# suoych/KEDs

Measured on AMD Instinct MI355X. Metric: query-images/sec (encode+0.5M top-10) ViT-L/14, higher is better.
Workload: dtype bf16/fp16 operands, fp32 accumulate; 1 GPU; ViT-L/14 encode_image (224x224 synthetic, random-init weights) + exact top-10 over a synthetic unit-norm 0.5M x 768 database; batch_per_gpu=128, global_batch=128, db_rows=500000, dim=768, k=10, parallelism=dp1 encoders + 1-way row-sharded scan

## Files before the change

### keds_amd/csrc/gemm.hip

```cpp
#include "keds_common.h"
#include <math.h>
#include "gemm_shared.h"
#include "gemm_quad_gen.h"

#ifndef KEDS_QUAD_AUX_X
#define KEDS_QUAD_AUX_X 0
#endif
#ifndef KEDS_QUAD_AUX_W
#define KEDS_QUAD_AUX_W 0
#endif

namespace {

constexpr int BM = 128, BN = 128, BK = 64;
constexpr int TILE_BYTES = 128 * BK * 2;
constexpr int BUF_BYTES = 2 * TILE_BYTES;


__device__ __forceinline__ float qgelu(float x) {
    return x * __builtin_amdgcn_rcpf(1.0f + __builtin_amdgcn_exp2f(-2.4554669595930157f * x));
}

template <int EPI>
__device__ __forceinline__ void epilogue_store(f32x4 v0, f32x4 v1, void* __restrict__ out, int m, int n, int N,
// ... 198 lines not shown
                if (m >= M) continue;
                if constexpr (epi_x3(EPI))
                    epilogue_store<epi_base(EPI)>(acc[2 * p][mi] * x3_ws + b0, acc[2 * p + 1][mi] * x3_ws + b1, out, m, n, N, aux, aux_i, ldc);
                else
                    epilogue_store<epi_base(EPI)>(acc[2 * p][mi] + b0, acc[2 * p + 1][mi] + b1, out, m, n, N, aux, aux_i, ldc, guard);
            }
        }
    }
}

template <int EPI>
constexpr int quad_nd() { return 18; }
template <int EPI, int ND = 0, int H = 0, int PSEL = -1>
__device__ __forceinline__ void pair_ln_epilogue(f32x4 (&acc)[4][8], const char* __restrict__ side, void* __restrict__ out,
                                                 int m0, int n0, int N, int wm, int wn, int g, int c,
                                                 void* __restrict__ aux2, u32x4* __restrict__ pend = nullptr, bool defer = false,
                                                 int* __restrict__ guard = nullptr) {
    float rstd[8], nmr[8];
    [[maybe_unused]] unsigned rmax = 0;
    int r0 = 128 * wm + c;
    asm volatile("" : "+v"(r0));
#pragma unroll
    for (int mi = 0; mi < 8; ++mi) {
        const f32x2 cf = *reinterpret_cast<const f32x2*>(side + (r0 + 16 * mi) * 8);
        rstd[mi] = cf[0];
        nmr[mi] = cf[1];
    }
    if (PSEL <= 0 && aux2 && n0 == 0 && wn == 0 && g == 0) {
        keds_stat_t* zero = reinterpret_cast<keds_stat_t*>(aux2) + 2 * (size_t)(m0 + r0);
#pragma unroll
        for (int mi = 0; mi < 8; ++mi) keds_stat_zero(zero + 32 * mi);
    }
    char* tile_out = reinterpret_cast<char*>(out) + ((size_t)m0 * N + n0) * 2;
#pragma unroll
    for (int p = 0; p < 2; ++p) {
        if (PSEL >= 0 && p != PSEL) continue;
        const int nl = 64 * wn + 32 * p + 8 * g;
        const f32x4 b0 = *reinterpret_cast<const f32x4*>(side + 2048 + nl * 4), b1 = *reinterpret_cast<const f32x4*>(side + 2048 + nl * 4 + 16);
        const f32x4 c0 = *reinterpret_cast<const f32x4*>(side + 3072 + nl * 4), c1 = *reinterpret_cast<const f32x4*>(side + 3072 + nl * 4 + 16);
#pragma unroll
        for (int mi = 0; mi < 8; ++mi) {
            f32x4 v0 = acc[2 * p][mi] * rstd[mi] + (c0 * nmr[mi] + b0);
            f32x4 v1 = acc[2 * p + 1][mi] * rstd[mi] + (c1 * nmr[mi] + b1);
            if constexpr (epi_qgelu(EPI)) {
                f32x4 z0 = v0 * -2.4554669595930157f, z1 = v1 * -2.4554669595930157f;
#pragma unroll
                for (int j = 0; j < 4; ++j) {
                    z0[j] = __builtin_amdgcn_exp2f(z0[j]);
                    z1[j] = __builtin_amdgcn_exp2f(z1[j]);
                }
                z0 = z0 + 1.0f;
                z1 = z1 + 1.0f;
#pragma unroll
                for (int j = 0; j < 4; ++j) {
                    z0[j] = __builtin_amdgcn_rcpf(z0[j]);
                    z1[j] = __builtin_amdgcn_rcpf(z1[j]);
                }
                v0 = v0 * z0;
                v1 = v1 * z1;
            }
            const unsigned off = ((unsigned)(r0 + 16 * mi) * (unsigned)N + (unsigned)nl) * 2u;
            u32x4 ov;
            if constexpr (epi_out_f16(EPI)) {
                rmax = f16_range_max(rmax, v0, v1);
                ov = __builtin_bit_cast(u32x4, f16x8{(f16_t)v0[0], (f16_t)v0[1], (f16_t)v0[2], (f16_t)v0[3],
                                                     (f16_t)v1[0], (f16_t)v1[1], (f16_t)v1[2], (f16_t)v1[3]});
            } else {
                ov = __builtin_bit_cast(u32x4, bf16x8{(bf16_t)v0[0], (bf16_t)v0[1], (bf16_t)v0[2], (bf16_t)v0[3],
                                                      (bf16_t)v1[0], (bf16_t)v1[1], (bf16_t)v1[2], (bf16_t)v1[3]});
            }
            if constexpr (ND > 0) {
                if (16 * H + p * 8 + mi >= 32 - ND && defer) {
                    pend[16 * H + p * 8 + mi - (32 - ND)] = ov;
                    continue;
                }
            }
            keds_store16<KEDS_ST_LN>(ov, tile_out, off);
        }
    }
    if constexpr (epi_out_f16(EPI)) f16_range_flag(guard, rmax);
}
template <int ND>
__device__ __forceinline__ void quad_flush_pending(const u32x4* __restrict__ pend, char* __restrict__ tile_out, int N, int wm, int wn2,
                                                   int g, int c, int i0, int i1) {
    int r0 = 128 * wm + c;
    asm volatile("" : "+v"(r0));
#pragma unroll
    for (int i = 0; i < ND; ++i) {
        if (i < i0 || i >= i1) continue;
        const int s_ = 32 - ND + i, h = s_ >> 4, p = (s_ >> 3) & 1, mi = s_ & 7;
        const unsigned off = ((unsigned)(r0 + 16 * mi) * (unsigned)N + (unsigned)(64 * (2 * wn2 + h) + 32 * p + 8 * g)) * 2u;
        keds_store16<KEDS_ST_LN>(pend[i], tile_out, off);
    }
}

template <bool REDUCE = true>
__device__ __forceinline__ void pair_resid_epilogue(f32x4 (&acc)[4][8], const char* __restrict__ side, void* __restrict__ out,
                                                    int m0, int n0, int N, int wm, int wn, int g, int c,
                                                    keds_stat_t* __restrict__ stats, char* __restrict__ red) {
    const int r0 = 128 * wm + c;
    char* tile = reinterpret_cast<char*>(out) + ((size_t)m0 * N + n0) * 2;
    const int nl = 64 * wn + 8 * g;
    f16x8 r[2][8];
#if KEDS_LD_RESID_AUX
    const auto trs = __builtin_amdgcn_make_buffer_rsrc(tile, 0, 0x7FFFFFFF, 0x00020000);
#endif
#pragma unroll
    for (int p = 0; p < 2; ++p)
#pragma unroll
        for (int mi = 0; mi < 8; ++mi) {
#if KEDS_LD_RESID_AUX
            r[p][mi] = __builtin_bit_cast(f16x8, __builtin_amdgcn_raw_buffer_load_b128(
                           trs, (int)(((unsigned)(r0 + 16 * mi) * (unsigned)N + (unsigned)(nl + 32 * p)) * 2u), 0, KEDS_LD_RESID_AUX));
#else
            r[p][mi] = *reinterpret_cast<const f16x8*>(tile + ((unsigned)(r0 + 16 * mi) * (unsigned)N + (unsigned)(nl + 32 * p)) * 2u);
#endif
        }
    f32x4 b[2][2];
#pragma unroll
    for (int p = 0; p < 2; ++p) {
        b[p][0] = *reinterpret_cast<const f32x4*>(side + 2048 + (nl + 32 * p) * 4);
        b[p][1] = *reinterpret_cast<const f32x4*>(side + 2048 + (nl + 32 * p) * 4 + 16);
    }
    f32x2* rw = reinterpret_cast<f32x2*>(red) + wn * 256 + r0;
#pragma unroll
    for (int mi = 0; mi < 8; ++mi) {
        f32x4 sv = f32x4{0.f, 0.f, 0.f, 0.f}, qv = sv;
#pragma unroll
        for (int p = 0; p < 2; ++p) {
            const f16x8 q = r[p][mi];
            const f32x4 v0 = f32x4{(float)q[0], (float)q[1], (float)q[2], (float)q[3]} + (acc[2 * p][mi] + b[p][0]);
            const f32x4 v1 = f32x4{(float)q[4], (float)q[5], (float)q[6], (float)q[7]} + (acc[2 * p + 1][mi] + b[p][1]);
            const f16x8 ov = f16x8{(f16_t)v0[0], (f16_t)v0[1], (f16_t)v0[2], (f16_t)v0[3], (f16_t)v1[0], (f16_t)v1[1], (f16_t)v1[2], (f16_t)v1[3]};
            keds_store16<KEDS_ST_RESID>(ov, tile, ((unsigned)(r0 + 16 * mi) * (unsigned)N + (unsigned)(nl + 32 * p)) * 2u);
            sv = sv + (v0 + v1);
            qv = qv + (v0 * v0 + v1 * v1);
        }
        float s = (sv[0] + sv[1]) + (sv[2] + sv[3]), ss = (qv[0] + qv[1]) + (qv[2] + qv[3]);
        s = rows_sum(s);
        ss = rows_sum(ss);
        if (stats && g == 0) rw[16 * mi] = f32x2{s, ss};
    }
    if constexpr (REDUCE) {
        if (stats) {
            __syncthreads();
            const int t = threadIdx.x;
            if (t < 256) {
                const f32x2* rr = reinterpret_cast<const f32x2*>(red) + t;
                const f32x2 a = rr[0], b = rr[256], c2 = rr[512], d = rr[768];
                keds_stat_add(stats + 2 * (size_t)(m0 + t), (a[0] + b[0]) + (c2[0] + d[0]), (a[1] + b[1]) + (c2[1] + d[1]));
            }
        }
    }
}

__device__ __forceinline__ void pair_resid_epilogue_acc(f32x4 (&acc)[4][8], void* __restrict__ out, int m0, int n0, int N,
                                                        int wm, int wn, int g, int c, keds_stat_t* __restrict__ stats,
                                                        char* __restrict__ red) {
    const int r0 = 128 * wm + c;
    char* tile = reinterpret_cast<char*>(out) + ((size_t)m0 * N + n0) * 2;
    const int nl = 64 * wn + 8 * g;
    f32x2* rw = reinterpret_cast<f32x2*>(red) + wn * 256 + r0;
#pragma unroll
    for (int mi = 0; mi < 8; ++mi) {
        float s = 0.f, ss = 0.f;
#pragma unroll
        for (int p = 0; p < 2; ++p) {
            const f32x4 v0 = acc[2 * p][mi], v1 = acc[2 * p + 1][mi];
            const f16x8 ov = f16x8{(f16_t)v0[0], (f16_t)v0[1], (f16_t)v0[2], (f16_t)v0[3], (f16_t)v1[0], (f16_t)v1[1], (f16_t)v1[2], (f16_t)v1[3]};
            *reinterpret_cast<f16x8*>(tile + ((unsigned)(r0 + 16 * mi) * (unsigned)N + (unsigned)(nl + 32 * p)) * 2u) = ov;
            s += sum8(v0, v1);
            ss += sum8(v0 * v0, v1 * v1);
        }
        s = rows_sum(s);
        ss = rows_sum(ss);
        if (stats && g == 0) rw[16 * mi] = f32x2{s, ss};
    }
    if (stats) {
        __syncthreads();
        const int t = threadIdx.x;
        if (t < 256) {
            const f32x2* rr = reinterpret_cast<const f32x2*>(red) + t;
            const f32x2 a = rr[0], b = rr[256], c2 = rr[512], d = rr[768];
            keds_stat_add(stats + 2 * (size_t)(m0 + t), (a[0] + b[0]) + (c2[0] + d[0]), (a[1] + b[1]) + (c2[1] + d[1]));
        }
    }
}

template <int N>
__device__ __forceinline__ void small_wait_barrier() {
    asm volatile("s_waitcnt vmcnt(%0)\n\ts_barrier" ::"n"(N) : "memory");
}
template <int MAXAHEAD>
__device__ __forceinline__ void small_wait_stage(int ahead) {
    if constexpr (MAXAHEAD == 0) {
        small_wait_barrier<0>();
    } else {
        if (ahead >= MAXAHEAD) small_wait_barrier<MAXAHEAD * 8>();
        else small_wait_stage<MAXAHEAD - 1>(ahead);
    }
}

template <int EPI, int NST>
__global__ __launch_bounds__(256, 2) void gemm_bt_kernel(const bf16_t* __restrict__ X, const bf16_t* __restrict__ W,
                                                         const float* __restrict__ bias, void* __restrict__ out,
                                                         int M, int N, int K, int n_tiles,
                                                         const float* __restrict__ aux, int aux_i,
                                                         float* __restrict__ part, int k_len, int tiles, int m_pad,
                                                         long long lda, long long ldc, void* __restrict__ aux2,
                                                         int* __restrict__ guard, long long a_plane, long long w_plane) {
    extern __shared__ __attribute__((aligned(16))) char smem[];
    const int bid_all = xcd_remap(blockIdx.x, gridDim.x);
    const int ks = part ? bid_all / tiles : 0;
    const int bid = part ? bid_all - ks * tiles : bid_all;
    const int k_begin = ks * k_len;
    const int tm = bid / n_tiles, tn = bid - tm * n_tiles;
    const int m0 = tm * BM, n0 = tn * BN;
    const int tid = threadIdx.x, lane = tid & 63;
    const int wave = __builtin_amdgcn_readfirstlane(tid >> 6);
    const int wn = wave >> 1, wm = wave & 1;
    const int g = lane >> 4, c = lane & 15;

    const int srow = lane >> 3, sslot = lane & 7;
    auto xrs_ = __builtin_amdgcn_make_buffer_rsrc(const_cast<void*>(static_cast<const void*>(X + (size_t)m0 * lda)), 0, 0x7FFFFFFF, 0x00020000);
    auto wrs_ = __builtin_amdgcn_make_buffer_rsrc(const_cast<void*>(static_cast<const void*>(W + (size_t)n0 * K)), 0, 0x7FFFFFFF, 0x00020000);
    int xsrc[4], wsrc[4];
#pragma unroll
    for (int i = 0; i < 4; ++i) {
        const int R = 32 * wave + 8 * i + srow;
        const int ch = sslot ^ swz_f(R);
        const int xr = m0 + R < M ? R : M - 1 - m0;
        xsrc[i] = (int)((long long)xr * lda * 2) + ch * 16;
        wsrc[i] = perm_w(R) * K * 2 + ch * 16;
    }
    auto stage = [&](int buf, int kt) {
        char* xb = smem + buf * BUF_BYTES + (32 * wave) * 128;
        char* wb = xb + TILE_BYTES;
        unsigned koff = (k_begin + kt * BK) * 2, kx = 0, kw = 0;
        if constexpr (epi_x3(EPI)) {
            const X3Seg sg = x3_seg(kt, K / BK);
            koff = sg.koff;
            kx = sg.a_lo ? (unsigned)(a_plane * 2) : 0u;
            kw = sg.w_lo ? (unsigned)(w_plane * 2) : 0u;
        }
#pragma unroll
        for (int i = 0; i < 4; ++i) {
            __builtin_amdgcn_raw_ptr_buffer_load_lds(xrs_, (__attribute__((address_space(3))) void*)(xb + i * 1024), 16, xsrc[i], koff + kx, 0, 0);
            __builtin_amdgcn_raw_ptr_buffer_load_lds(wrs_, (__attribute__((address_space(3))) void*)(wb + i * 1024), 16, wsrc[i], koff + kw, 0, 0);
        }
    };

    int xoff[2], woff[2];
    {
        const int xr = 64 * wm + c, wr = 64 * wn + c;
#pragma unroll
        for (int kk = 0; kk < 2; ++kk) {
            xoff[kk] = xr * 128 + (((4 * kk + g) ^ swz_f(xr)) << 4);
            woff[kk] = TILE_BYTES + wr * 128 + (((4 * kk + g) ^ swz_f(wr)) << 4);
        }
    }

    f32x4 acc[4][4];
#pragma unroll
    for (int ni = 0; ni < 4; ++ni)
#pragma unroll
        for (int mi = 0; mi < 4; ++mi) acc[ni][mi] = f32x4{0.f, 0.f, 0.f, 0.f};

    const int nk = (epi_x3(EPI) ? 3 : 1) * ((part ? k_len : K) / BK);
#pragma unroll
    for (int s = 0; s < NST; ++s)
        if (s < nk) stage(s, s);
    {
        int ahead = nk - 1;
        if (ahead > NST - 1) ahead = NST - 1;
        small_wait_stage<NST - 1>(ahead);
    }
    bf16x8 xa[4], wa[4], xb[4], wb[4];
#pragma unroll
    for (int i = 0; i < 4; ++i) {
        xa[i] = *reinterpret_cast<const bf16x8*>(smem + xoff[0] + i * 2048);
        wa[i] = *reinterpret_cast<const bf16x8*>(smem + woff[0] + i * 2048);
    }
#define KEDS_SMALL_MFMA(xc, wc, xn, wn_, nb, kkn, PREFETCH)                                                    \
    {                                                                                                          \
        _Pragma("unroll") for (int mi = 0; mi < 4; ++mi) {                                                     \
            _Pragma("unroll") for (int ni = 0; ni < 4; ++ni)                                                   \
                acc[ni][mi] = mma<epi_f16(EPI)>(wc[ni], xc[mi], acc[ni][mi]);   \
            if (PREFETCH) {                                                                                    \
                xn[mi] = *reinterpret_cast<const bf16x8*>((nb) + xoff[kkn] + mi * 2048);                       \
                wn_[mi] = *reinterpret_cast<const bf16x8*>((nb) + woff[kkn] + mi * 2048);                      \
            }                                                                                                  \
        }                                                                                                      \
        if (PREFETCH) {                                                                                        \
            KEDS_SM_G KEDS_SM_G KEDS_SM_G KEDS_SM_G                                                            \
        }                                                                                                      \
    }
#define KEDS_SM_G                                                                                              \
    __builtin_amdgcn_sched_group_barrier(0x008, 4, 0);                                                         \
    __builtin_amdgcn_sched_group_barrier(0x100, 2, 0);

    int slot = 0;
    for (int kt = 0; kt < nk; ++kt) {
        const char* cb = smem + slot * BUF_BYTES;
        int nslot = slot + 1 == NST ? 0 : slot + 1;
        const char* ob = smem + nslot * BUF_BYTES;
        __builtin_amdgcn_sched_barrier(0);
// ... 453 lines not shown
    };
    auto side_write = [&](char* side, int n0_) {
        if constexpr (epi_resid16(EPI)) *reinterpret_cast<float*>(side + 2048 + tid * 4) = pb;
        if constexpr (epi_is_ln(EPI)) {
            float rs, nm;
            ln_coeff_from((keds_stat_t)(((unsigned long long)st_raw[1] << 32) | st_raw[0]),
                          (keds_stat_t)(((unsigned long long)st_raw[3] << 32) | st_raw[2]), 1.0f / (float)K, rs, nm,
                          n0_ == 0 ? guard : nullptr);
            *reinterpret_cast<f32x2*>(side + tid * 8) = f32x2{rs, nm};
            *reinterpret_cast<float*>(side + 2048 + tid * 4) = pb;
            *reinterpret_cast<float*>(side + 3072 + tid * 4) = pc;
        }
    };

    int id = blockIdx.x;
    int tm, tn;
    quad_tile_coords(xcd_remap(id, ntiles), m_tiles, n_tiles, tm, tn);
    int m0 = tm * TM, n0 = tn * TN;
    xrs = make_rs(X + (size_t)m0 * K);
    wrs = make_rs(W + (size_t)n0 * K);
    side_request(m0, n0);
#pragma unroll
    for (int q = 0; q < 16; ++q) issue(0, q);
#pragma unroll
    for (int q = 0; q < 16; ++q) issue(1, q);
    if constexpr (epi_is_ln(EPI)) asm volatile("s_waitcnt vmcnt(32)" : "+v"(st_raw), "+v"(pb), "+v"(pc)::"memory");
    if constexpr (epi_resid16(EPI)) asm volatile("s_waitcnt vmcnt(32)" : "+v"(pb)::"memory");
    side_write(smem + qd::SIDE0, n0);
    asm volatile("s_waitcnt vmcnt(16) lgkmcnt(0)\n\ts_barrier" ::: "memory");

    constexpr int QUAD_ND = quad_nd<EPI>();
    constexpr int QUAD_PS = (QUAD_ND + 5) / 6;
    [[maybe_unused]] u32x4 pend[QUAD_ND];
    [[maybe_unused]] char* pend_base = nullptr;
    [[maybe_unused]] bool have_pend = false;
    constexpr bool DEFER = PERSIST && epi_is_ln(EPI) && !epi_qgelu(EPI);
    for (int it = 0;; ++it) {
        char* side = smem + qd::SIDE0 + (it & 1) * 4096;
        const int nid = id + step;
        const bool more = PERSIST && nid < ntiles;
        int nm0 = 0, nn0 = 0;
        if (more) {
            int ntm, ntn;
            quad_tile_coords(xcd_remap(nid, ntiles), m_tiles, n_tiles, ntm, ntn);
            nm0 = ntm * TM;
            nn0 = ntn * TN;
        }
        bf16x8 xa[8], wa[8], xb[8], wb[8];
#pragma unroll
        for (int j = 0; j < 8; ++j) wa[j] = *reinterpret_cast<const bf16x8*>(smem + wrow + slot0 + j * 2048);
#pragma unroll
        for (int mi = 0; mi < 8; ++mi) xa[mi] = *reinterpret_cast<const bf16x8*>(smem + xrow + slot0 + mi * 2048);

        KEDS_QUAD_STEP(true, xa, wa, xb, wb, smem, slot1, false, false, 0, true)
        int p = 0;
        if constexpr (DEFER) {
            if (have_pend) {
#define KEDS_QUAD_PEEL(pp, SY)                                                                                          \
    {                                                                                                                   \
        const char* ob = smem + (((pp) + 1) & 1) * PBUF_BYTES;                                                          \
        KEDS_QUAD_STEP(false, xb, wb, xa, wa, ob, slot0, SY, true, (pp) + 2, true)                                      \
        quad_flush_pending<QUAD_ND>(pend, pend_base, N, wm, wn2, g, c, 2 * QUAD_PS * (pp), 2 * QUAD_PS * (pp) + QUAD_PS); \
        KEDS_QUAD_STEP(false, xa, wa, xb, wb, ob, slot1, false, false, 0, true)                                         \
        quad_flush_pending<QUAD_ND>(pend, pend_base, N, wm, wn2, g, c, 2 * QUAD_PS * (pp) + QUAD_PS, 2 * QUAD_PS * (pp) + 2 * QUAD_PS); \
    }
                KEDS_QUAD_PEEL(0, 1)
                KEDS_QUAD_PEEL(1, 2 * QUAD_PS)
                KEDS_QUAD_PEEL(2, 2 * QUAD_PS)
                KEDS_QUAD_PEEL(3, 2 * QUAD_PS)
#undef KEDS_QUAD_PEEL
                p = 4;
                have_pend = false;
            }
        }
        for (; p + 2 < np; ++p) {
            const char* ob = smem + ((p + 1) & 1) * PBUF_BYTES;
            KEDS_QUAD_STEP(false, xb, wb, xa, wa, ob, slot0, true, true, p + 2, true)
            KEDS_QUAD_STEP(false, xa, wa, xb, wb, ob, slot1, false, false, 0, true)
        }
        {
            const char* ob = smem + ((p + 1) & 1) * PBUF_BYTES;
            KEDS_QUAD_STEP(false, xb, wb, xa, wa, ob, slot0, true, false, 0, true)
            KEDS_QUAD_STEP(false, xa, wa, xb, wb, ob, slot1, false, false, 0, true)
            KEDS_QUAD_STEP(false, xb, wb, xa, wa, ob, slot0, false, false, 0, false)
        }

        if (more) {
            asm volatile("s_waitcnt lgkmcnt(0)\n\ts_barrier" ::: "memory");
            if constexpr (epi_is_ln(EPI)) {
                st_raw = *reinterpret_cast<const u32x4*>(reinterpret_cast<const keds_stat_t*>(aux) + 2 * (size_t)(nm0 + tid));
                pb = bias[nn0 + tid];
                pc = bias[N + nn0 + tid];
            }
            if constexpr (epi_resid16(EPI)) pb = bias ? bias[nn0 + tid] : 0.f;
            xrs = make_rs(X + (size_t)nm0 * K);
            wrs = make_rs(W + (size_t)nn0 * K);
#pragma unroll
            for (int q = 0; q < 16; ++q) issue(0, q);
#pragma unroll
            for (int q = 0; q < 16; ++q) issue(1, q);
        }

        [[maybe_unused]] const bool defer_now = more && aux_i != 0 && np >= 8;
        KEDS_QUAD_DRAIN
        f32x4 av[4][8];
        [[maybe_unused]] keds_stat_t* stats = reinterpret_cast<keds_stat_t*>(const_cast<float*>(aux));
        [[maybe_unused]] char* red = smem + qd::RED_OFF;
#define KEDS_QUAD_EPI(h)                                                                                               \
    if constexpr (epi_is_ln(EPI))                                                                                      \
        pair_ln_epilogue<EPI>(av, side, out, m0, n0, N, wm, 2 * wn2 + h, g, c, aux2, nullptr, false, guard);        \
    else if constexpr (epi_resid16(EPI))                                                                \
        pair_resid_epilogue<false>(av, side, out, m0, n0, N, wm, 2 * wn2 + h, g, c, stats, red);                    \
    else                                                                                                               \
        tile_epilogue<EPI, 8>(av, bias, out, m0 + 128 * wm + c, M, n0 + 64 * (2 * wn2 + h) + 8 * g, N, K, aux, aux_i, aux2, N, g == 0, guard, \
                              epi_x3(EPI) ? x3_wscale(w_plane) : 1.0f);
        if constexpr (DEFER) {
#define KEDS_QUAD_EPQ(h, p)                                                                                             \
    KEDS_QUAD_READ_Q##h##p(av)                                                                                          \
    pair_ln_epilogue<EPI, QUAD_ND, h, p>(av, side, out, m0, n0, N, wm, 2 * wn2 + h, g, c, aux2, pend, defer_now, guard); \
    __builtin_amdgcn_sched_barrier(0);
            KEDS_QUAD_EPQ(0, 0)
            KEDS_QUAD_EPQ(0, 1)
            KEDS_QUAD_EPQ(1, 0)
            KEDS_QUAD_EPQ(1, 1)
#undef KEDS_QUAD_EPQ
        } else {
            KEDS_QUAD_READ_HALF0(av)
            KEDS_QUAD_EPI(0)
            __builtin_amdgcn_sched_barrier(0);
            KEDS_QUAD_READ_HALF1(av)
            KEDS_QUAD_EPI(1)
        }
#undef KEDS_QUAD_EPI
        if constexpr (DEFER) {
            have_pend = defer_now;
            pend_base = reinterpret_cast<char*>(out) + ((size_t)m0 * N + n0) * 2;
        }
        if constexpr (epi_resid16(EPI)) {
            if (stats) {
                __syncthreads();
                const f32x2* rr = reinterpret_cast<const f32x2*>(red) + tid;
                const f32x2 a = rr[0], b = rr[256], c2 = rr[512], d = rr[768];
                keds_stat_add(stats + 2 * (size_t)(m0 + tid), (a[0] + b[0]) + (c2[0] + d[0]), (a[1] + b[1]) + (c2[1] + d[1]));
            }
        }
        if (!more) break;
        id = nid;
        m0 = nm0;
        n0 = nn0;
        side_write(smem + qd::SIDE0 + ((it + 1) & 1) * 4096, n0);
        asm volatile("s_waitcnt vmcnt(0) lgkmcnt(0)\n\ts_barrier" ::: "memory");
    }
}
template <int EPI>
__global__ __launch_bounds__(256, 1) void gemm_bt_quad3_kernel(const bf16_t* __restrict__ X, const bf16_t* __restrict__ W,
                                                               const float* __restrict__ bias, void* __restrict__ out,
                                                               int M, int N, int K, int n_tiles,
                                                               const float* __restrict__ aux, int ntiles) {
    static_assert(epi_resid16(EPI), "three-deep A ring: residual epilogue only");
    using namespace pr;
    extern __shared__ __attribute__((aligned(16))) char smem[];
    constexpr int WRING = 3 * OP_BYTES;
    const int m_tiles = ntiles / n_tiles;
    const int tid = threadIdx.x, lane = tid & 63;
    const int wave = __builtin_amdgcn_readfirstlane(tid >> 6);
    const int wn2 = wave & 1, wm = wave >> 1;
    const int g = lane >> 4, c = lane & 15;
    const int R0 = 8 * wave + (lane >> 3);
    const int sch = (lane & 7) ^ swz_f(R0);
    const unsigned xoff = (unsigned)R0 * (unsigned)K * 2u + sch * 16;
    const unsigned woff = (unsigned)perm_w(R0) * (unsigned)K * 2u + sch * 16;
    const unsigned rstride = 32u * (unsigned)K * 2u;
    int tm, tn;
    quad_tile_coords(xcd_remap(blockIdx.x, ntiles), m_tiles, n_tiles, tm, tn);
    const int m0 = tm * TM, n0 = tn * TN;
    auto xrs = make_rs(X + (size_t)m0 * K);
    auto wrs = make_rs(W + (size_t)n0 * K);
    auto issue_a = [&](int kt, int buf, int i) {
        char* dst = smem + buf * OP_BYTES + (wave + 4 * i) * 1024;
        __builtin_amdgcn_raw_ptr_buffer_load_lds(xrs, (__attribute__((address_space(3))) void*)dst, 16, xoff,
                                                 i * rstride + (unsigned)kt * (TK * 2), 0, KEDS_LD_A3_AUX);
    };
    auto issue_w = [&](int kt, int buf, int i) {
        char* dst = smem + WRING + buf * OP_BYTES + (wave + 4 * i) * 1024;
        __builtin_amdgcn_raw_ptr_buffer_load_lds(wrs, (__attribute__((address_space(3))) void*)dst, 16, woff,
                                                 i * rstride + (unsigned)kt * (TK * 2), 0, 0);
    };
    int wfree = 0, afree = 0;
    auto issue = [&](int ip, int q) {
        if (q < 8) issue_w(ip, wfree, q);
        else issue_a(ip + 1, afree, q - 8);
    };
    const int f = (c >> 1) & 7;
    const int slot0 = ((0 + g) ^ f) << 4, slot1 = ((4 + g) ^ f) << 4;
    const int xrow = (128 * wm + c) * 128;
    const int wrow0 = (128 * wn2 + c) * 128;
    const int np = K / TK;
    float pb = 0.f;
    if (bias) {
        const float* bp = bias + n0 + tid;
        asm volatile("global_load_dword %0, %1, off" : "=v"(pb) : "v"(bp) : "memory");
    }
#pragma unroll
    for (int i = 0; i < 8; ++i) issue_a(0, 0, i);
#pragma unroll
    for (int i = 0; i < 8; ++i) issue_w(0, 0, i);
#pragma unroll
    for (int i = 0; i < 8; ++i) issue_a(1, 1, i);
#pragma unroll
    for (int i = 0; i < 8; ++i) issue_w(1, 1, i);
#pragma unroll
    for (int i = 0; i < 8; ++i) issue_a(2, 2, i);
    asm volatile("s_waitcnt vmcnt(40)" : "+v"(pb)::"memory");
    asm volatile("s_waitcnt vmcnt(24) lgkmcnt(0)\n\ts_barrier" ::: "memory");
    bf16x8 xa[8], wa[8], xb[8], wb[8];
#pragma unroll
    for (int j = 0; j < 8; ++j) wa[j] = *reinterpret_cast<const bf16x8*>(smem + WRING + wrow0 + slot0 + j * 2048);
#pragma unroll
    for (int mi = 0; mi < 8; ++mi) xa[mi] = *reinterpret_cast<const bf16x8*>(smem + xrow + slot0 + mi * 2048);

    int ia = 0, iw = 0, wrow = WRING + wrow0;
    {
        const char* ab = smem;
        KEDS_QUAD_STEP(true, xa, wa, xb, wb, ab, slot1, false, 0, 0, true)
    }
    int p = 0;
    for (; p + 3 < np; ++p) {
        const int ia1 = ia == 2 ? 0 : ia + 1, iw1 = iw ^ 1;
        asm volatile("s_waitcnt vmcnt(8) lgkmcnt(0)\n\ts_barrier" ::: "memory");
        wfree = iw;
        afree = ia;
        {
            const char* ab = smem + ia1 * OP_BYTES;
            wrow = WRING + (iw1 - ia1) * OP_BYTES + wrow0;
            KEDS_QUAD_STEP(false, xb, wb, xa, wa, ab, slot0, false, 1, p + 2, true)
            KEDS_QUAD_STEP(false, xa, wa, xb, wb, ab, slot1, false, 0, 0, true)
        }
        ia = ia1;
        iw = iw1;
    }
    {
        const int ia1 = ia == 2 ? 0 : ia + 1, iw1 = iw ^ 1;
        asm volatile("s_waitcnt vmcnt(8) lgkmcnt(0)\n\ts_barrier" ::: "memory");
        wfree = iw;
        const char* ab = smem + ia1 * OP_BYTES;
        wrow = WRING + (iw1 - ia1) * OP_BYTES + wrow0;
        KEDS_QUAD_STEP(false, xb, wb, xa, wa, ab, slot0, false, 2, p + 2, true)
        KEDS_QUAD_STEP(false, xa, wa, xb, wb, ab, slot1, false, 0, 0, true)
        ia = ia1;
        iw = iw1;
    }
    {
        const int ia1 = ia == 2 ? 0 : ia + 1, iw1 = iw ^ 1;
        asm volatile("s_waitcnt vmcnt(0) lgkmcnt(0)\n\ts_barrier" ::: "memory");
        const char* ab = smem + ia1 * OP_BYTES;
        wrow = WRING + (iw1 - ia1) * OP_BYTES + wrow0;
        KEDS_QUAD_STEP(false, xb, wb, xa, wa, ab, slot0, false, 0, 0, true)
        KEDS_QUAD_STEP(false, xa, wa, xb, wb, ab, slot1, false, 0, 0, true)
        KEDS_QUAD_STEP(false, xb, wb, xa, wa, ab, slot0, false, 0, 0, false)
    }
    asm volatile("s_waitcnt lgkmcnt(0)\n\ts_barrier" ::: "memory");
    char* side = smem + WRING;
    char* red = smem + WRING + 8192;
    *reinterpret_cast<float*>(side + 2048 + tid * 4) = pb;
    __syncthreads();
    KEDS_QUAD_DRAIN
    f32x4 av[4][8];
    keds_stat_t* stats = reinterpret_cast<keds_stat_t*>(const_cast<float*>(aux));
    KEDS_QUAD_READ_HALF0(av)
    pair_resid_epilogue<false>(av, side, out, m0, n0, N, wm, 2 * wn2 + 0, g, c, stats, red);
    __builtin_amdgcn_sched_barrier(0);
    KEDS_QUAD_READ_HALF1(av)
    pair_resid_epilogue<false>(av, side, out, m0, n0, N, wm, 2 * wn2 + 1, g, c, stats, red);
    if (stats) {
        __syncthreads();
        const f32x2* rr = reinterpret_cast<const f32x2*>(red) + tid;
        const f32x2 a = rr[0], b = rr[256], c2 = rr[512], d = rr[768];
        keds_stat_add(stats + 2 * (size_t)(m0 + tid), (a[0] + b[0]) + (c2[0] + d[0]), (a[1] + b[1]) + (c2[1] + d[1]));
    }
}

#undef make_rs
#undef KEDS_QUAD_STEP
#undef KEDS_QUAD_GROUP
#undef KEDS_QG2
#undef KEDS_QGAP
#undef KEDS_QRD
#undef KEDS_QMFMA





GemmSwitches& gemm_switches() {
    static GemmSwitches sw;
    return sw;
}

struct GemmLaunchRecord {
    int form[2], ring[2], splits[2], persistent, flags;
    void info(int out[8]) const {
        const int v[8] = {form[0], form[1], ring[0], ring[1], splits[0], splits[1], persistent, flags};
        for (int i = 0; i < 8; ++i) out[i] = v[i];
    }
};
thread_local GemmLaunchRecord tl_rec = {};
thread_local int tl_rec_slot = 0;
inline void rec_launch(int form, int ring, int splits, int persistent = 0, int flags = 0) {
    tl_rec.form[tl_rec_slot] = form;
    tl_rec.ring[tl_rec_slot] = ring;
    tl_rec.splits[tl_rec_slot] = splits;
    if (tl_rec_slot == 0) {
        tl_rec.persistent = persistent;
        tl_rec.flags = flags;
    }
}

struct GemmArgs {
    const void *A, *W;
    const float* bias;
    void* out;
    int M, N, K;
    const float* aux;
    int aux_i;
    void* aux2;
    long long lda, ldc;
    hipStream_t st;
    long long a_plane, w_plane;
    float* splitk;
};

template <int EPI, int NST>
int launch_small(const GemmArgs& a, const GemmPlan::Part&) {
    if (int rc = keds_func_lds_once((const void*)gemm_bt_kernel<EPI, NST>, NST * BUF_BYTES, "gemm_bt_kernel")) return rc;
    const int m_tiles = (a.M + BM - 1) / BM, n_tiles = a.N / BN;
    const int tiles = m_tiles * n_tiles;
    rec_launch(KEDS_GEMM_FORM_SMALL, NST, 1);
    KEDS_LAUNCH((gemm_bt_kernel<EPI, NST>), tiles, 256, NST * BUF_BYTES, a.st, (const bf16_t*)a.A, (const bf16_t*)a.W, a.bias, a.out, a.M, a.N,
                a.K, n_tiles, a.aux, a.aux_i, (float*)nullptr, 0, tiles, 0, a.lda, a.ldc, a.aux2, keds_numerics_guard(), a.a_plane, a.w_plane);
    return keds_check_launch("gemm_bt_kernel");
}

template <int EPI, int NST>
int launch_splitk(const GemmArgs& a, const GemmPlan::Part& p) {
    if (int rc = keds_func_lds_once((const void*)gemm_bt_kernel<EPI, NST>, NST * BUF_BYTES, "gemm_bt_kernel")) return rc;
    const int m_tiles = (a.M + BM - 1) / BM, n_tiles = a.N / BN;
    const int tiles = m_tiles * n_tiles, splits = p.splits;
    const int m_pad = m_tiles * BM;
    rec_launch(KEDS_GEMM_FORM_SMALL, NST, splits);
    KEDS_LAUNCH((gemm_bt_kernel<EPI, NST>), tiles * splits, 256, NST * BUF_BYTES, a.st, (const bf16_t*)a.A, (const bf16_t*)a.W, a.bias, a.out,
                a.M, a.N, a.K, n_tiles, a.aux, a.aux_i, a.splitk, a.K / splits, tiles, m_pad, a.lda, a.ldc, a.aux2, (int*)nullptr, 0LL, 0LL);
    if (int rc = keds_check_launch("gemm_bt_kernel(split-K)")) return rc;
    const int threads = a.M * (a.N / 8);
    KEDS_LAUNCH((gemm_splitk_reduce_kernel<EPI>), (threads + 255) / 256, 256, 0, a.st, (const float*)a.splitk, splits, m_pad, a.bias, a.out, a.M,
                a.N, a.K, a.aux, a.aux_i, a.ldc, a.aux2, keds_numerics_guard());
    return keds_check_launch("gemm_splitk_reduce_kernel");
}

template <int EPI>
int launch_pair(const GemmArgs& a, const GemmPlan::Part& p) {
    const int m_tiles = a.M / pr::TM, n_tiles = a.N / pr::TN;
    if constexpr (epi_resid16(EPI)) {
        if (p.flags & KEDS_GEMM_FLAG_RESID_PROLOGUE) {
            if (int rc = keds_func_lds_once((const void*)gemm_bt_pair_kernel<EPI, 1>, pr::LDS_BYTES, "gemm_bt_pair_kernel")) return rc;
            rec_launch(KEDS_GEMM_FORM_PAIR, 2, 1, 0, KEDS_GEMM_FLAG_RESID_PROLOGUE);
            KEDS_LAUNCH((gemm_bt_pair_kernel<EPI, 1>), m_tiles * n_tiles, 512, pr::LDS_BYTES, a.st, (const bf16_t*)a.A, (const bf16_t*)a.W,
                        a.bias, a.out, a.M, a.N, a.K, n_tiles, a.aux, a.aux_i, a.aux2, keds_numerics_guard(), 0LL, 0LL);
            return keds_check_launch("gemm_bt_pair_kernel");
        }
    }
    if (int rc = keds_func_lds_once((const void*)gemm_bt_pair_kernel<EPI>, pr::LDS_BYTES, "gemm_bt_pair_kernel")) return rc;
    rec_launch(KEDS_GEMM_FORM_PAIR, 2, 1);
    KEDS_LAUNCH((gemm_bt_pair_kernel<EPI>), m_tiles * n_tiles, 512, pr::LDS_BYTES, a.st, (const bf16_t*)a.A, (const bf16_t*)a.W, a.bias, a.out,
                a.M, a.N, a.K, n_tiles, a.aux, a.aux_i, a.aux2, keds_numerics_guard(), a.a_plane, a.w_plane);
    return keds_check_launch("gemm_bt_pair_kernel");
}

template <int EPI>
int launch_quad(const GemmArgs& a, const GemmPlan::Part&) {
    const int n_tiles = a.N / pr::TN, ntiles = (a.M / pr::TM) * n_tiles;
    if (int rc = keds_func_lds_once((const void*)gemm_bt_quad_kernel<EPI>, qd::LDS_BYTES, "gemm_bt_quad_kernel")) return rc;
    rec_launch(KEDS_GEMM_FORM_QUAD, 2, 1);
    KEDS_LAUNCH((gemm_bt_quad_kernel<EPI>), ntiles, 256, qd::LDS_BYTES, a.st, (const bf16_t*)a.A, (const bf16_t*)a.W, a.bias, a.out, a.M, a.N,
                a.K, n_tiles, a.aux, a.aux_i, a.aux2, keds_numerics_guard(), ntiles, a.a_plane, a.w_plane);
    return keds_check_launch("gemm_bt_quad_kernel");
}

template <int EPI>
int launch_quad_persistent(const GemmArgs& a, const GemmPlan::Part& p) {
    const int n_tiles = a.N / pr::TN, ntiles = (a.M / pr::TM) * n_tiles;
    if (int rc = keds_func_lds_once((const void*)gemm_bt_quad_kernel<EPI, 1>, qd::LDS_BYTES, "gemm_bt_quad_kernel")) return rc;
    const int aux_i = epi_is_ln(EPI) ? p.defer : a.aux_i;
    rec_launch(KEDS_GEMM_FORM_QUAD, 2, 1, 1, epi_is_ln(EPI) && !epi_qgelu(EPI) && aux_i && a.K / pr::TK >= 8 ? KEDS_GEMM_FLAG_DEFER : 0);
    KEDS_LAUNCH((gemm_bt_quad_kernel<EPI, 1>), p.workgroups, 256, qd::LDS_BYTES, a.st, (const bf16_t*)a.A, (const bf16_t*)a.W, a.bias, a.out,
                a.M, a.N, a.K, n_tiles, a.aux, aux_i, a.aux2, keds_numerics_guard(), ntiles, a.a_plane, a.w_plane);
    return keds_check_launch("gemm_bt_quad_kernel<persistent>");
}

template <int EPI>
int launch_quad3(const GemmArgs& a, const GemmPlan::Part&) {
    const int n_tiles = a.N / pr::TN, ntiles = (a.M / pr::TM) * n_tiles;
    if (int rc = keds_func_lds_once((const void*)gemm_bt_quad3_kernel<EPI>, 5 * pr::OP_BYTES, "gemm_bt_quad3_kernel")) return rc;
    rec_launch(KEDS_GEMM_FORM_QUAD3, 3, 1);
    KEDS_LAUNCH((gemm_bt_quad3_kernel<EPI>), ntiles, 256, 5 * pr::OP_BYTES, a.st, (const bf16_t*)a.A, (const bf16_t*)a.W, a.bias, a.out, a.M,
                a.N, a.K, n_tiles, a.aux, ntiles);
    return keds_check_launch("gemm_bt_quad3_kernel");
}

template <int EPI>
int launch_part(const GemmArgs& a, const GemmPlan::Part& p) {
    switch (p.form) {
        case KEDS_GEMM_FORM_SMALL:
            if (p.splits > 1) return p.ring == 4 ? launch_splitk<EPI, 4>(a, p) : launch_splitk<EPI, 2>(a, p);
            return p.ring == 4 ? launch_small<EPI, 4>(a, p) : launch_small<EPI, 2>(a, p);
        case KEDS_GEMM_FORM_PAIR: return launch_pair<EPI>(a, p);
        case KEDS_GEMM_FORM_QUAD: return p.persistent ? launch_quad_persistent<EPI>(a, p) : launch_quad<EPI>(a, p);
        case KEDS_GEMM_FORM_QUAD3:
            if constexpr (epi_resid16(EPI)) return launch_quad3<EPI>(a, p);
            else break;
        default: break;
    }
    keds_set_error("keds_gemm_bt: no kernel of form %d for epilogue %d", p.form, EPI);
    return KEDS_E_LAUNCH;
}

template <int EPI>
int launch_gemm(GemmArgs a) {
    const int M = a.M, N = a.N, K = a.K;
    KedsProfScope prof(KEDS_PROF_GEMM, a.st,  true);
    prof.work(2.0 * M * N * K);
    tl_rec = GemmLaunchRecord{};
    tl_rec_slot = 0;
    const GemmSwitches& sw = gemm_switches();
    const GemmPlanNeeds needs = gemm_plan_needs(EPI, M, N, K, a.lda, a.ldc, sw);
    size_t splitk_bytes = 0;
    if (needs.splitk) keds_splitk_scratch(&a.splitk, &splitk_bytes);
    if (!a.splitk) splitk_bytes = 0;
    const GemmPlan plan = gemm_plan(EPI, M, N, K, a.lda, a.ldc, needs.cus ? keds_device_cus() : 0, splitk_bytes, false, sw);

    a.M = plan.main.rows;
    if (int rc = launch_part<EPI>(a, plan.main)) return rc;
    if (plan.tail.form != KEDS_GEMM_FORM_NONE) {
        tl_rec_slot = 1;
        const size_t m_main = plan.main.rows;
        const size_t esz = (epi_base(EPI) == KEDS_EPI_BIAS_RESID_F32 || epi_base(EPI) == KEDS_EPI_BIAS_F32 || EPI == KEDS_EPI_RESID_STATS_F32)
                               ? 4 : 2;
        if constexpr (epi_is_ln(EPI)) {
            a.aux = (const float*)((const keds_stat_t*)a.aux + 2 * m_main);
            if (a.aux2) a.aux2 = (keds_stat_t*)a.aux2 + 2 * m_main;
        } else if constexpr (EPI == KEDS_EPI_RESID_STATS_F32) {
            a.aux = (const float*)((const keds_stat_t*)a.aux + 2 * m_main);
            a.aux2 = (char*)a.aux2 + m_main * N * 2;
        } else if constexpr (epi_resid16(EPI)) {
            if (a.aux) a.aux = (const float*)((const keds_stat_t*)a.aux + 2 * m_main);
        }
        a.A = (const char*)a.A + m_main * K * 2;
        a.out = (char*)a.out + m_main * N * esz;
        a.M = plan.tail.rows;
        if (int rc = launch_part<EPI>(a, plan.tail)) return rc;
    }
    int want[8], got[8];
    plan.info(want);
    tl_rec.info(got);
    for (int i = 0; i < 8; ++i) {
        if (got[i] != want[i]) {
            keds_set_error("keds_gemm_bt: launched form differs from the plan at [%d]: %d, planned %d (epilogue %d, %d x %d x %d)", i, got[i],
                           want[i], EPI, M, N, K);
            return KEDS_E_LAUNCH;
        }
    }
    return KEDS_OK;
}

}

bool keds_gemm_splits_rows(int M, int N, int K) { return gemm_big_tiles_fill(M, N, K, gemm_switches()) && M % 256 != 0; }

extern "C" int keds_gemm_last_launch(int* info) {
    KEDS_REQUIRE(info, "keds_gemm_last_launch: null pointer");
    tl_rec.info(info);
    return KEDS_OK;
}

extern "C" int keds_gemm_force_small(int on) {
    for (const int bit : {8, 13, 14, 15})
        KEDS_REQUIRE(!((on >> bit) & 1), "keds_gemm_force_small: bit %d is no longer offered", bit);
    gemm_switches() = gemm_switches_decode(on, GemmSwitches{});
    return KEDS_OK;
}

static int gemm_check_shape(const char* who, int M, int N, int K, int64_t lda, int64_t ldc, int epilogue) {
    KEDS_REQUIRE(M > 0 && N > 0 && K > 0, "%s: empty problem", who);
    KEDS_REQUIRE(N % BN == 0, "%s: N=%d must be a multiple of %d", who, N, BN);
    KEDS_REQUIRE(K % BK == 0, "%s: K=%d must be a multiple of %d", who, K, BK);
    KEDS_REQUIRE(lda >= K && ldc >= N && lda % 8 == 0 && ldc % 8 == 0, "%s: bad row strides", who);
    KEDS_REQUIRE(epi_base(epilogue) != KEDS_EPI_PATCH_F32 || ldc == N, "%s: EPI_PATCH needs a dense output", who);
    return KEDS_OK;
}

extern "C" int keds_gemm_plan_query(int epilogue, int M, int N, int K, int64_t lda, int64_t ldc, int cus, size_t splitk_bytes,
                                    int small_lds, int* info) {
    KEDS_REQUIRE(info, "keds_gemm_plan_query: null pointer");
    KEDS_REQUIRE(epilogue >= 0 && epilogue <= KEDS_EPI_BIAS_F32_H, "keds_gemm_plan_query: unknown epilogue %d", epilogue);
    if (int rc = gemm_check_shape("keds_gemm_plan_query", M, N, K, lda, ldc, epilogue)) return rc;
    gemm_plan(epilogue, M, N, K, lda, ldc, cus, splitk_bytes, small_lds != 0, gemm_switches()).info(info);
    return KEDS_OK;
}

extern "C" int keds_gemm_plan_query_many(int64_t n, const int64_t* cases, int* info) {
    KEDS_REQUIRE(n >= 0 && (n == 0 || (cases && info)), "keds_gemm_plan_query_many: bad argument");
    for (int64_t i = 0; i < n; ++i) {
        const int64_t* c = cases + 9 * i;
        if (int rc = keds_gemm_plan_query((int)c[0], (int)c[1], (int)c[2], (int)c[3], c[4], c[5], (int)c[6], (size_t)c[7], (int)c[8], info + 8 * i))
            return rc;
    }
    return KEDS_OK;
}

extern "C" int keds_gemm_bt_ex2(const void* A, int64_t lda, const void* W, const float* bias, void* out, int64_t ldc,
                                int M, int N, int K, int epilogue, const float* aux, int aux_i, void* aux2, void* stream) {
    KEDS_REQUIRE(A && W && out, "keds_gemm_bt: null pointer");
    if (int rc = gemm_check_shape("keds_gemm_bt", M, N, K, lda, ldc, epilogue)) return rc;
    if (epi_base(epilogue) == KEDS_EPI_PATCH_F32) KEDS_REQUIRE(aux && aux_i > 0, "keds_gemm_bt: EPI_PATCH needs the positional embedding and G");
    if (epi_is_ln(epilogue)) KEDS_REQUIRE(bias && aux, "keds_gemm_bt: EPI_LN_* needs bias = [bias' | colsum] and aux = row statistics");
    if (epilogue == KEDS_EPI_RESID_STATS_F32) KEDS_REQUIRE(aux && aux2, "keds_gemm_bt: EPI_RESID_STATS needs aux = statistics and aux2 = bf16 copy");
    if (epilogue == KEDS_EPI_BIAS_BF16_HEADF32)
        KEDS_REQUIRE(aux && aux_i >= 0, "keds_gemm_bt: EPI_BIAS_BF16_HEADF32 needs the fp32 head buffer and its row count");
    if (epi_x3(epilogue)) {
        keds_set_error("keds_gemm_bt: split-operand epilogues go through keds_gemm_x3");
        return KEDS_E_ARG;
    }
    const GemmArgs g{A, W, bias, out, M, N, K, aux, aux_i, aux2, lda, ldc, (hipStream_t)stream, 0, 0, nullptr};
#define KEDS_GEMM_CASE(E) case E: return launch_gemm<E>(g);
    switch (epilogue) {
        KEDS_GEMM_CASE(KEDS_EPI_BIAS_BF16)
        KEDS_GEMM_CASE(KEDS_EPI_BIAS_QGELU_BF16)
        KEDS_GEMM_CASE(KEDS_EPI_BIAS_RELU_BF16)
        KEDS_GEMM_CASE(KEDS_EPI_BIAS_RESID_F32)
        KEDS_GEMM_CASE(KEDS_EPI_BIAS_F32)
        KEDS_GEMM_CASE(KEDS_EPI_PATCH_F32)
        KEDS_GEMM_CASE(KEDS_EPI_LN_BIAS_BF16)
        KEDS_GEMM_CASE(KEDS_EPI_LN_QGELU_BF16)
        KEDS_GEMM_CASE(KEDS_EPI_RESID_STATS_F32)
        KEDS_GEMM_CASE(KEDS_EPI_RESID_STATS_F16)
        KEDS_GEMM_CASE(KEDS_EPI_LN_BIAS_BF16_H)
        KEDS_GEMM_CASE(KEDS_EPI_LN_QGELU_BF16_H)
        KEDS_GEMM_CASE(KEDS_EPI_BIAS_BF16_HEADF32)
        KEDS_GEMM_CASE(KEDS_EPI_LN_BIAS_F16_H)
        KEDS_GEMM_CASE(KEDS_EPI_LN_QGELU_F16_H)
        KEDS_GEMM_CASE(KEDS_EPI_RESID_STATS_F16_H)
        KEDS_GEMM_CASE(KEDS_EPI_BIAS_RESID_F32_H)
        KEDS_GEMM_CASE(KEDS_EPI_BIAS_QGELU_F16_H)
        KEDS_GEMM_CASE(KEDS_EPI_PATCH_F32_H)
        KEDS_GEMM_CASE(KEDS_EPI_BIAS_F32_H)
        default: keds_set_error("keds_gemm_bt: unknown epilogue %d", epilogue); return KEDS_E_ARG;
    }
#undef KEDS_GEMM_CASE
}

extern "C" int keds_gemm_x3(const void* a, int64_t a_plane, int64_t lda, const void* w, int64_t w_plane, const float* bias, void* out,
                            int64_t ldc, int M, int N, int K, int epilogue, int aux_i, int w_exp, void* stream) {
    KEDS_REQUIRE(a && w && out && M > 0 && N > 0 && K > 0, "keds_gemm_x3: bad argument");
    KEDS_REQUIRE(N % BN == 0 && K % BK == 0 && lda >= K && ldc >= N && lda % 8 == 0 && ldc % 8 == 0, "keds_gemm_x3: bad shape / strides");
    KEDS_REQUIRE(a_plane > 0 && w_plane > 0 && a_plane * 2 + 256LL * lda * 2 < (1LL << 31) && w_plane * 2 + 256LL * K * 2 < (1LL << 31),
                 "keds_gemm_x3: plane strides out of range");
    KEDS_REQUIRE(w_exp >= -100 && w_exp <= 100, "keds_gemm_x3: w_exp %d out of range", w_exp);
    const GemmArgs g{a, w, bias, out, M, N, K, nullptr, epilogue == KEDS_EPI_X3_QGELU_PAIR ? aux_i : 0, nullptr, lda, ldc, (hipStream_t)stream,
                     a_plane, x3_pack_wplane(w_plane, w_exp), nullptr};
    switch (epilogue) {
        case KEDS_EPI_X3_BIAS_F32: return launch_gemm<KEDS_EPI_X3_BIAS_F32>(g);
        case KEDS_EPI_X3_RESID_F32: return launch_gemm<KEDS_EPI_X3_RESID_F32>(g);
        case KEDS_EPI_X3_QGELU_PAIR:
            KEDS_REQUIRE(aux_i > 0, "keds_gemm_x3: KEDS_EPI_X3_QGELU_PAIR needs the output planes' stride");
            return launch_gemm<KEDS_EPI_X3_QGELU_PAIR>(g);
        default: keds_set_error("keds_gemm_x3: epilogue %d is not a split-operand epilogue", epilogue); return KEDS_E_ARG;
    }
}

extern "C" int keds_gemm_bt_ex(const void* A, int64_t lda, const void* W, const float* bias, void* out, int64_t ldc,
                               int M, int N, int K, int epilogue, const float* aux, int aux_i, void* stream) {
    return keds_gemm_bt_ex2(A, lda, W, bias, out, ldc, M, N, K, epilogue, aux, aux_i, nullptr, stream);
}

extern "C" int keds_gemm_bt(const void* A, const void* W, const float* bias, void* out, int M, int N, int K,
                            int epilogue, const float* aux, int aux_i, void* stream) {
    return keds_gemm_bt_ex2(A, K, W, bias, out, N, M, N, K, epilogue, aux, aux_i, nullptr, stream);
}
```

Measured before the change: 6709 query-images/sec.

## Prefetch residual tiles during final MFMA steps of quad3 GEMM epilogue

The three-deep-ring residual GEMM kernel now issues the buffer loads for the fp16 residual tile inside the last K-loop steps, using the step macro's issue slots. The epilogue is rewritten row by row, adding bias, residual and accumulator in registers, storing, and computing row statistics, with waits placed so the second half's loads can still be in flight while the first half is processed. The intent is to hide residual-read latency that the old epilogue exposed after the main loop. It adds 32 u32x4 registers of live state, which risks spills at one block per CU. Optional timestamp instrumentation is also added behind a compile flag.

Result: no change. 6730 query-images/sec (median of 6 runs) (+0.3%).

```diff
diff --git a/keds_amd/csrc/gemm.hip b/keds_amd/csrc/gemm.hip
--- a/keds_amd/csrc/gemm.hip
+++ b/keds_amd/csrc/gemm.hip
@@ -374,6 +374,25 @@
             }
         }
     }
+}
+
+__device__ __forceinline__ void quad3_resid_row(const f32x4 (&av)[4], u32x4 q0, u32x4 q1, const f32x4 (&b)[2][2], char* __restrict__ tile,
+                                                unsigned off, bool write_stats, f32x2* __restrict__ rw) {
+    f32x4 sv = f32x4{0.f, 0.f, 0.f, 0.f}, qv = sv;
+#pragma unroll
+    for (int p = 0; p < 2; ++p) {
+        const f16x8 q = __builtin_bit_cast(f16x8, p ? q1 : q0);
+        const f32x4 v0 = f32x4{(float)q[0], (float)q[1], (float)q[2], (float)q[3]} + (av[2 * p] + b[p][0]);
+        const f32x4 v1 = f32x4{(float)q[4], (float)q[5], (float)q[6], (float)q[7]} + (av[2 * p + 1] + b[p][1]);
+        const f16x8 ov = f16x8{(f16_t)v0[0], (f16_t)v0[1], (f16_t)v0[2], (f16_t)v0[3], (f16_t)v1[0], (f16_t)v1[1], (f16_t)v1[2], (f16_t)v1[3]};
+        keds_store16<KEDS_ST_RESID == 0 ? 8 : KEDS_ST_RESID>(ov, tile, off + 64u * p);
+        sv = sv + (v0 + v1);
+        qv = qv + (v0 * v0 + v1 * v1);
+    }
+    float s = (sv[0] + sv[1]) + (sv[2] + sv[3]), ss = (qv[0] + qv[1]) + (qv[2] + qv[3]);
+    s = rows_sum(s);
+    ss = rows_sum(ss);
+    if (write_stats) *rw = f32x2{s, ss};
 }
 
 __device__ __forceinline__ void pair_resid_epilogue_acc(f32x4 (&acc)[4][8], void* __restrict__ out, int m0, int n0, int N,
@@ -1133,6 +1152,22 @@
         asm volatile("s_waitcnt vmcnt(0) lgkmcnt(0)\n\ts_barrier" ::: "memory");
     }
 }
+#ifdef KEDS_QUAD3_STAMPS
+__device__ unsigned long long* keds_q3_stamp_buf = nullptr;
+#define KEDS_Q3_STAMP(i)                                                                                                \
+    {                                                                                                                   \
+        __builtin_amdgcn_sched_barrier(0);                                                                              \
+        q3_stamp[i] = __builtin_amdgcn_s_memtime();                                                                     \
+        __builtin_amdgcn_sched_barrier(0);                                                                              \
+    }
+#define KEDS_Q3_STAMP_WAIT(i, n)                                                                                        \
+    __builtin_amdgcn_sched_barrier(0);                                                                                  \
+    asm volatile("s_waitcnt vmcnt(" #n ")" ::: "memory");                                                               \
+    KEDS_Q3_STAMP(i)
+#else
+#define KEDS_Q3_STAMP(i)
+#define KEDS_Q3_STAMP_WAIT(i, n)
+#endif
 template <int EPI>
 __global__ __launch_bounds__(256, 1) void gemm_bt_quad3_kernel(const bf16_t* __restrict__ X, const bf16_t* __restrict__ W,
                                                                const float* __restrict__ bias, void* __restrict__ out,
@@ -1140,6 +1175,10 @@
                                                                const float* __restrict__ aux, int ntiles) {
     static_assert(epi_resid16(EPI), "three-deep A ring: residual epilogue only");
     using namespace pr;
+#ifdef KEDS_QUAD3_STAMPS
+    unsigned long long q3_stamp[8] = {};
+#endif
+    KEDS_Q3_STAMP(0)
     extern __shared__ __attribute__((aligned(16))) char smem[];
     constexpr int WRING = 3 * OP_BYTES;
     const int m_tiles = ntiles / n_tiles;
@@ -1182,6 +1221,12 @@
         const float* bp = bias + n0 + tid;
         asm volatile("global_load_dword %0, %1, off" : "=v"(pb) : "v"(bp) : "memory");
     }
+    char* tile = reinterpret_cast<char*>(out) + ((size_t)m0 * N + n0) * 2;
+    const auto trs = make_rs(tile);
+    const unsigned rlane = ((unsigned)(128 * wm + c) * (unsigned)N + (unsigned)(128 * wn2 + 8 * g)) * 2u;
+    auto resid_off = [&](int h, int q) { return rlane + ((unsigned)(16 * (q >> 1)) * (unsigned)N + (unsigned)(64 * h + 32 * (q & 1))) * 2u; };
+    auto resid_request = [&](int h, int q) { return __builtin_bit_cast(u32x4, __builtin_amdgcn_raw_buffer_load_b128(trs, (int)resid_off(h, q), 0, KEDS_LD_RESID_AUX)); };
+    u32x4 rq[2][16];
 #pragma unroll
     for (int i = 0; i < 8; ++i) issue_a(0, 0, i);
 #pragma unroll
@@ -1236,30 +1281,70 @@
         asm volatile("s_waitcnt vmcnt(0) lgkmcnt(0)\n\ts_barrier" ::: "memory");
         const char* ab = smem + ia1 * OP_BYTES;
         wrow = WRING + (iw1 - ia1) * OP_BYTES + wrow0;
-        KEDS_QUAD_STEP(false, xb, wb, xa, wa, ab, slot0, false, 0, 0, true)
+        {
+            auto issue = [&](int, int q) { rq[0][q] = resid_request(0, q); };
+            KEDS_QUAD_STEP(false, xb, wb, xa, wa, ab, slot0, false, 1, 0, true)
+        }
         KEDS_QUAD_STEP(false, xa, wa, xb, wb, ab, slot1, false, 0, 0, true)
-        KEDS_QUAD_STEP(false, xb, wb, xa, wa, ab, slot0, false, 0, 0, false)
-    }
+        {
+            auto issue = [&](int, int q) { rq[1][q] = resid_request(1, q); };
+            KEDS_QUAD_STEP(false, xb, wb, xa, wa, ab, slot0, false, 1, 0, false)
+        }
+    }
+    __builtin_amdgcn_sched_barrier(0);
+    KEDS_Q3_STAMP(1)
     asm volatile("s_waitcnt lgkmcnt(0)\n\ts_barrier" ::: "memory");
     char* side = smem + WRING;
     char* red = smem + WRING + 8192;
     *reinterpret_cast<float*>(side + 2048 + tid * 4) = pb;
-    __syncthreads();
+    asm volatile("s_waitcnt lgkmcnt(0)\n\ts_barrier" ::: "memory");
     KEDS_QUAD_DRAIN
-    f32x4 av[4][8];
     keds_stat_t* stats = reinterpret_cast<keds_stat_t*>(const_cast<float*>(aux));
-    KEDS_QUAD_READ_HALF0(av)
-    pair_resid_epilogue<false>(av, side, out, m0, n0, N, wm, 2 * wn2 + 0, g, c, stats, red);
-    __builtin_amdgcn_sched_barrier(0);
-    KEDS_QUAD_READ_HALF1(av)
-    pair_resid_epilogue<false>(av, side, out, m0, n0, N, wm, 2 * wn2 + 1, g, c, stats, red);
+#define KEDS_Q3_ROW(h, mi)                                                                                              \
+    {                                                                                                                   \
+        f32x4 av[4];                                                                                                    \
+        KEDS_QUAD_READ_G##h##mi(av)                                                                                     \
+        quad3_resid_row(av, rq[h][2 * (mi)], rq[h][2 * (mi) + 1], bs, tile, resid_off(h, 2 * (mi)), stats && g == 0,    \
+                        reinterpret_cast<f32x2*>(red) + (2 * wn2 + (h)) * 256 + 128 * wm + c + 16 * (mi));              \
+        __builtin_amdgcn_sched_barrier(0);                                                                              \
+    }
+#define KEDS_Q3_HALF(h)                                                                                                 \
+    {                                                                                                                   \
+        f32x4 bs[2][2];                                                                                                 \
+        _Pragma("unroll") for (int p = 0; p < 2; ++p) {                                                                 \
+            const int nl = 64 * (2 * wn2 + (h)) + 8 * g + 32 * p;                                                       \
+            bs[p][0] = *reinterpret_cast<const f32x4*>(side + 2048 + nl * 4);                                           \
+            bs[p][1] = *reinterpret_cast<const f32x4*>(side + 2048 + nl * 4 + 16);                                      \
+        }                                                                                                               \
+        KEDS_Q3_ROW(h, 0) KEDS_Q3_ROW(h, 1) KEDS_Q3_ROW(h, 2) KEDS_Q3_ROW(h, 3)                                         \
+        KEDS_Q3_ROW(h, 4) KEDS_Q3_ROW(h, 5) KEDS_Q3_ROW(h, 6) KEDS_Q3_ROW(h, 7)                                         \
+    }
+    KEDS_Q3_STAMP_WAIT(2, 16)
+    KEDS_Q3_HALF(0)
+    KEDS_Q3_STAMP(3)
+    KEDS_Q3_STAMP_WAIT(4, 16)
+    KEDS_Q3_HALF(1)
+    KEDS_Q3_STAMP(5)
+#undef KEDS_Q3_HALF
+#undef KEDS_Q3_ROW
     if (stats) {
-        __syncthreads();
+        asm volatile("s_waitcnt lgkmcnt(0)\n\ts_barrier" ::: "memory");
         const f32x2* rr = reinterpret_cast<const f32x2*>(red) + tid;
         const f32x2 a = rr[0], b = rr[256], c2 = rr[512], d = rr[768];
         keds_stat_add(stats + 2 * (size_t)(m0 + tid), (a[0] + b[0]) + (c2[0] + d[0]), (a[1] + b[1]) + (c2[1] + d[1]));
     }
-}
+#ifdef KEDS_QUAD3_STAMPS
+    asm volatile("s_waitcnt vmcnt(0)" ::: "memory");
+    KEDS_Q3_STAMP(6)
+    if (keds_q3_stamp_buf && lane == 0) {
+        unsigned long long* sb = keds_q3_stamp_buf + ((size_t)blockIdx.x * 4 + wave) * 8;
+#pragma unroll
+        for (int i = 0; i < 7; ++i) sb[i] = q3_stamp[i];
+    }
+#endif
+}
+#undef KEDS_Q3_STAMP
+#undef KEDS_Q3_STAMP_WAIT
 
 #undef make_rs
 #undef KEDS_QUAD_STEP
@@ -1456,6 +1541,13 @@
 }
 
 bool keds_gemm_splits_rows(int M, int N, int K) { return gemm_big_tiles_fill(M, N, K, gemm_switches()) && M % 256 != 0; }
+
+#ifdef KEDS_QUAD3_STAMPS
+extern "C" int keds_quad3_stamps_set(void* buf) {
+    unsigned long long* p = static_cast<unsigned long long*>(buf);
+    return hipMemcpyToSymbol(HIP_SYMBOL(keds_q3_stamp_buf), &p, sizeof(p)) == hipSuccess ? KEDS_OK : KEDS_E_LAUNCH;
+}
+#endif
 
 extern "C" int keds_gemm_last_launch(int* info) {
     KEDS_REQUIRE(info, "keds_gemm_last_launch: null pointer");
```
